# ArashMehraban/CeedPetscSolid

Hardware: AMD Instinct MI355X
Metric: MDoF/s for matrix-free Jacobian apply, p=4 hyperFS hex, 1/2/4/8 GPU (higher is better)
Workload: dtype f64; 1 GPU; config 4: hyperFS, hollow cylinder 10x110x90 = 99000 hex per GPU (stand-in for cylinder8_99Ke_4ss_us.exo), degree 4, Q=5, clamped ends, Jacobian apply y=J(u)x; global_dofs=19429080, elements_per_gpu=99000, ldofs_per_gpu=19537320, halo_dofs_rank0=0, assembly=pipelined: 2 segments on 2 streams, last segment 16384 elements, schedule=static, partition=single GPU

## Files before the change

ceedpetscsolid_amd/csrc/ceed_core.cpp:

```cpp
#include "ceed_impl.hpp"
#include "kernels_pointblock.hpp"

using namespace cps;

static int g_err_return = 0;
static thread_local char g_err_msg[1024] = "";

int ceed_error(const char *fmt, ...) {
  va_list ap;
  va_start(ap, fmt);
  vsnprintf(g_err_msg, sizeof g_err_msg, fmt, ap);
  va_end(ap);
  if (!g_err_return) {
    fprintf(stderr, "[ceed mi355x] error: %s\n", g_err_msg);
    abort();
  }
  return 1;
}
extern "C" int CeedXSetErrorReturn(int enable) { g_err_return = enable; return 0; }
extern "C" const char *CeedXLastError(void) { return g_err_msg; }

static CeedVector_private s_vec_active, s_vec_none;
static CeedElemRestriction_private s_rstr_none;
static CeedBasis_private s_basis_colloc;
static CeedQFunction_private s_qf_none;
static CeedRequest s_req_immediate, s_req_ordered;
extern "C" {
const CeedVector CEED_VECTOR_ACTIVE = &s_vec_active;
const CeedVector CEED_VECTOR_NONE = &s_vec_none;
const CeedElemRestriction CEED_ELEMRESTRICTION_NONE = &s_rstr_none;
const CeedBasis CEED_BASIS_COLLOCATED = &s_basis_colloc;
const CeedQFunction CEED_QFUNCTION_NONE = &s_qf_none;
CeedRequest *const CEED_REQUEST_IMMEDIATE = &s_req_immediate;
CeedRequest *const CEED_REQUEST_ORDERED = &s_req_ordered;
const CeedInt CEED_STRIDES_BACKEND[3] = {-1, -1, -1};
const char *const CeedMemTypes[] = {"host", "device"};
}

static int env_int(const char *name, int dflt) { const char *e = getenv(name); return e && *e ? atoi(e) : dflt; }
static bool env_is(const char *name, const char *val) { const char *e = getenv(name); return e && !strcmp(e, val); }

extern "C" int CeedInit(const char *resource, Ceed *ceed) {
  if (!resource || strncmp(resource, "/gpu/hip", 8))
    return ceed_error("this library serves /gpu/hip/mi355x only (got '%s'); there is no CPU path",
                      resource ? resource : "(null)");
  int ndev = 0;
  hipError_t e = hipGetDeviceCount(&ndev);
  if (e != hipSuccess || ndev < 1)
    return ceed_error("no HIP device visible (%s): the MI355X backend cannot run",
                      e != hipSuccess ? hipGetErrorString(e) : "device count 0");
  Ceed c = new Ceed_private;
  c->resource = "/gpu/hip/mi355x";
  HIPCHK(hipGetDevice(&c->device));
  CeedOptions &o = c->opt;
  o.recompute_geo = !env_is("CEED_MI355X_GEO", "0");
  o.direct_interior = !env_is("CEED_MI355X_DIRECT", "0");
  o.affine_geo = !env_is("CEED_MI355X_AFFINE", "0");
  o.swept_geo = !env_is("CEED_MI355X_SWEPT", "0");
  o.derived_state = !env_is("CEED_MI355X_DERIVED", "0");
  if (env_is("CEED_MI355X_ASSEMBLE", "serial")) o.pipe_segments = 0;
  else { const int ps = env_int("CEED_MI355X_PIPE_SEGMENTS", 0); o.pipe_segments = ps >= 2 ? std::min(ps, 16) : -1; }
  o.pipe_mb = std::max(0, env_int("CEED_MI355X_PIPE_MB", o.pipe_mb));
  o.pipe_min_total_rounds = std::max(0, env_int("CEED_MI355X_PIPE_MIN_TOTAL", o.pipe_min_total_rounds));
  o.pipe_min_rounds = std::max(0, env_int("CEED_MI355X_PIPE_MIN_ROUNDS", o.pipe_min_rounds));
  o.pencil_waves = std::max(0, env_int("CEED_MI355X_PENCIL_WAVES", 0));
  o.ovl_mode = env_int("CEED_MI355X_OVL_MODE", o.ovl_mode);
  o.ovl_groups0 = std::max(0, env_int("CEED_MI355X_OVL_G0", o.ovl_groups0));
  o.ovl_groups1 = std::max(0, env_int("CEED_MI355X_OVL_G1", o.ovl_groups1));
  o.comm_priority = env_int("CEED_MI355X_COMM_PRIO", o.comm_priority);
  o.comm_inline = env_int("CEED_MI355X_COMM_INLINE", o.comm_inline);
  o.fold_pack = env_int("CEED_MI355X_FOLD_PACK", o.fold_pack);
  *ceed = c;
  return 0;
}
void ceed_ref(Ceed c) { c->refcount++; }
int (*g_rccl_comm_destroy)(void *) = nullptr;
static void ceed_free_parked(Ceed c) {
  for (void *p : c->parked) (void)hipFree(p);
  c->parked.clear();
}
void ceed_retire(Ceed c, void *p) {
  if (!p) return;
  if (c->capturing || c->live_graphs > 0) c->parked.push_back(p);
  else { (void)hipStreamSynchronize(c->stream); (void)hipFree(p); }
}
void ceed_unref(Ceed c) {
  if (--c->refcount > 0) return;
  if (c->comm) {
    if (c->comm_stream) (void)hipStreamSynchronize(c->comm_stream);
    if (g_rccl_comm_destroy) g_rccl_comm_destroy(c->comm);
  }
  if (c->comm_stream) (void)hipStreamDestroy(c->comm_stream);
  if (c->capture_stream) (void)hipStreamDestroy(c->capture_stream);
  if (c->side_stream) (void)hipStreamDestroy(c->side_stream);
  c->evec.release();
  ceed_free_parked(c);
  if (c->ev_fork) (void)hipEventDestroy(c->ev_fork);
  if (c->ev_join) (void)hipEventDestroy(c->ev_join);
  for (hipEvent_t ev : c->ev_seg) if (ev) (void)hipEventDestroy(ev);
  if (c->h_scalar) (void)hipHostFree(c->h_scalar);
  delete c;
}
int ceed_need_side_stream(Ceed c) {
  if (c->side_stream) return 0;
  HIPCHK(hipStreamCreateWithFlags(&c->side_stream, hipStreamNonBlocking));
  HIPCHK(hipEventCreateWithFlags(&c->ev_fork, hipEventDisableTiming));
  HIPCHK(hipEventCreateWithFlags(&c->ev_join, hipEventDisableTiming));
  return 0;
}
extern "C" int CeedDestroy(Ceed *ceed) {
  if (!ceed || !*ceed) return 0;
  ceed_unref(*ceed);
  *ceed = nullptr;
  return 0;
}
extern "C" int CeedGetResource(Ceed ceed, const char **resource) { *resource = ceed->resource.c_str(); return 0; }
extern "C" int CeedGetPreferredMemType(Ceed, CeedMemType *type) { *type = CEED_MEM_DEVICE; return 0; }
extern "C" int CeedXSetStream(Ceed ceed, void *s) { ceed->stream = (hipStream_t)s; return 0; }
extern "C" int CeedXSynchronize(Ceed ceed) {
  if (ceed->capturing) return ceed_error("CeedXSynchronize during graph capture");
  HIPCHK(hipStreamSynchronize(ceed->stream));
  return 0;
}
extern "C" int CeedXClockProbe(Ceed ceed, int spin_us, double *ghz) {
  if (ceed->capturing) return ceed_error("CeedXClockProbe during graph capture");
  if (spin_us < 1 || spin_us > 1000000) return ceed_error("CeedXClockProbe: 1 us ... 1 s");
  struct Stream { hipStream_t s = nullptr; ~Stream() { if (s) (void)hipStreamDestroy(s); } } ps;
  DevArray<long long> d;
  long long h[2] = {0, 0};
  HIPCHK(hipStreamCreateWithFlags(&ps.s, hipStreamNonBlocking));
  CHK(d.alloc(nullptr, 2));
  HIPCHK(launch_clock_probe(d.get(), spin_us, ps.s));
  HIPCHK(hipMemcpyAsync(h, d.get(), sizeof h, hipMemcpyDeviceToHost, ps.s));
  HIPCHK(hipStreamSynchronize(ps.s));
  *ghz = h[1] > 0 ? (double)h[0] / ((double)h[1] * 10.0) : 0.;
  return 0;
}
static void release_capture_deps(Ceed ceed) {
  std::vector<GraphDep> deps;
  deps.swap(ceed->capture_deps);
  for (GraphDep &d : deps) { CeedVector v = d.v; (void)CeedVectorDestroy(&v); }
}
extern "C" int CeedXGraphBeginCapture(Ceed ceed) {
  if (ceed->capturing) return ceed_error("graph capture already in progress");
  HIPCHK(hipStreamSynchronize(ceed->stream));
  if (!ceed->capture_stream) HIPCHK(hipStreamCreateWithFlags(&ceed->capture_stream, hipStreamNonBlocking));
  ceed->saved_stream = ceed->stream;
  ceed->stream = ceed->capture_stream;
  HIPCHK(hipStreamBeginCapture(ceed->stream, hipStreamCaptureModeRelaxed));
  ceed->capturing = true;
  release_capture_deps(ceed);
  return 0;
}
extern "C" int CeedXGraphEndCapture(Ceed ceed, CeedXGraph *graph) {
// ... 363 lines not shown
```

ceedpetscsolid_amd/csrc/ceed_impl.hpp:

```cpp
#pragma once
#include <ceed.h>
#include <hip/hip_runtime_api.h>

#include <algorithm>
#include <cmath>
#include <cstdarg>
#include <cstdio>
#include <cstdlib>
#include <cstring>
#include <memory>
#include <string>
#include <vector>

#include "dev_array.hpp"
#include "kernels.hpp"

int ceed_error(const char *fmt, ...);
#define CHK(x) do { int ierr_ = (x); if (ierr_) return ierr_; } while (0)
#define HIPCHK(x) do { hipError_t e_ = (x); if (e_ != hipSuccess) \
  return ceed_error("%s failed: %s (%s:%d)", #x, hipGetErrorString(e_), __FILE__, __LINE__); } while (0)

struct CeedOptions {
  bool recompute_geo = true;
  bool direct_interior = true;
  bool derived_state = true;
  bool affine_geo = true;
  bool swept_geo = true;
  int pipe_segments = -1;
  int pipe_mb = 0;
  int pipe_min_total_rounds = 20;
  int pipe_min_rounds = 4;
  int pencil_waves = 0;
  int ovl_mode = 0;
  int ovl_groups0 = 1, ovl_groups1 = 0;
  int fold_pack = 1;
  int comm_inline = 1;
  int comm_priority = 0;
};

struct GraphDep { CeedVector v; const double *geo; const double *derived; };
struct Ceed_private {
  int refcount = 1;
  std::string resource;
  hipStream_t stream = nullptr;
  int device = 0;
  CeedOptions opt;
  DevArray<double> evec;
  std::vector<void *> parked;
  int live_graphs = 0;
  hipStream_t side_stream = nullptr;
  hipEvent_t ev_fork = nullptr, ev_join = nullptr;
  hipEvent_t ev_seg[16] = {nullptr};
  void *comm = nullptr;
  int comm_rank = 0, comm_size = 1;
  hipStream_t comm_stream = nullptr;
  DevArray<double> d_scalar;
  double *h_scalar = nullptr;
  DevArray<int> d_pb_bad;
  hipStream_t capture_stream = nullptr, saved_stream = nullptr;
  bool capturing = false;
  std::vector<GraphDep> capture_deps;
};
struct CeedXGraph_private {
  std::vector<GraphDep> deps;
  Ceed ceed = nullptr;
  hipGraph_t graph = nullptr;
  hipGraphExec_t exec = nullptr;
  size_t nodes = 0;
};

struct CeedVector_private {
  Ceed ceed = nullptr;
  int refcount = 1;
  CeedInt length = 0;
  double *h = nullptr, *d = nullptr;
  uint64_t version = 0;
  bool h_owned = false, d_owned = false;
  bool h_valid = false, d_valid = false;
  DevArray<double> geo;
  DevArray<double> geo_aff;
  DevArray<double> geo_swept;
  int geo_axis = 0;
  int geo_nelem = 0, geo_Q = 0;
  double geo_qref[cps::MAXN1D] = {0}, geo_qwt[cps::MAXN1D] = {0};
  DevArray<double> derived;
  bool derived_valid = false;
  int derived_nelem = 0, derived_Q3 = 0;
  double derived_nu = 0., derived_E = 0.;
};

struct RowMap {
  std::vector<uint32_t> h_node_off;
  DevArray<uint32_t> d_rowptr, d_cols, d_node_off;
  int nrows = 0;
  cps::NodeMap view() const { return cps::NodeMap{d_rowptr.get(), d_cols.get(), d_node_off.get(), nrows, 0}; }
};
struct CsrMap : RowMap {
  bool built = false, full_cover = false;
  int nprio = 0, nskipped = 0;
  std::vector<uint32_t> h_rowptr, h_cols;
};
struct PipeMap : RowMap {
  int E = 0, req_seg = 0, waves = 0, mb = 0;
  const CsrMap *base = nullptr;
  int nseg = 0;
  std::vector<int> elem_bound, row_bound;
};

struct CeedElemRestriction_private {
  Ceed ceed = nullptr;
  int refcount = 1;
  CeedInt nelem = 0, elemsize = 0, ncomp = 0, compstride = 0, lsize = 0;
  bool strided = false, backend_strides = true;
  CeedInt strides[3] = {0, 0, 0};
  std::vector<CeedInt> h_offsets;
  DevArray<uint32_t> d_offsets;
  CsrMap csr;
  CsrMap csr_shell;
  std::vector<std::unique_ptr<PipeMap>> pipes;
  int interior_private = 0;
  DevArray<uint32_t> d_int_off;
  int int_per_elem = 0;
};

struct CeedBasis_private {
  Ceed ceed = nullptr;
  int refcount = 1;
  CeedInt dim = 3, ncomp = 0, P1d = 0, Q1d = 0;
  CeedQuadMode qmode = CEED_GAUSS;
  std::vector<double> interp1d, grad1d, qref1d, qweight1d, colo1d;
};

struct QFField { std::string name; CeedInt size; CeedEvalMode emode; };

struct CeedQFunction_private {
  Ceed ceed = nullptr;
  int refcount = 1;
  CeedQFunctionUser f = nullptr;
  std::string source, name;
  int kind = cps::QF_NONE;
  void *ctx = nullptr;
  size_t ctxsize = 0;
  CeedInt identity_size = 0;
  std::vector<QFField> in, out;
};

struct OpField { bool set = false; CeedElemRestriction rstr = nullptr; CeedBasis basis = nullptr; CeedVector vec = nullptr; };

enum PlanKind { PLAN_NONE = 0, PLAN_FUSED_GRAD, PLAN_SETUP_GEO, PLAN_PROLONG, PLAN_RESTRICT, PLAN_COORD, PLAN_ENERGY };

struct CeedXHalo_private;

struct CeedOperator_private {
  Ceed ceed = nullptr;
  int refcount = 1;
  CeedQFunction qf = nullptr;
  std::vector<OpField> in, out;
  bool composite = false;
  std::vector<CeedOperator> sub;
  int plan = PLAN_NONE;
  int i_active = -1, i_qdata = -1, i_state = -1, i_weight = -1, o_active = -1, o_state = -1, o_qdata = -1;
  cps::BasisTables tables;
  double eo[6][cps::EO_TAB];
  std::string kernel_name;
  bool kernel_fused = false;
  std::string kernel_name_full;
  int geo_mode = 0;
  DevArray<uint32_t> d_off_flagged;
  std::vector<std::pair<const RowMap *, DevArray<unsigned char>>> row_flags;
  struct PackFold { const RowMap *M; CeedXHalo H; long serial; DevArray<uint32_t> d_ptr, d_slot; bool ok; };
  std::vector<PackFold> pack_folds;
  std::vector<unsigned char> h_mask;
  int mask_mode = 0;
  CeedVector scale = nullptr;
  std::vector<unsigned char> h_mask_fine;
  DevArray<uint32_t> d_own_f;
  bool own_full_cover = false;
  DevArray<double> d_w;
  bool w_ready = false, w_unit = false;
  CeedVector w_scale = nullptr;
  uint64_t w_version = 0;
  int ovl_lead = 0;
  CsrMap ovl_csr;
  long ovl_halo_checked = 0;
  bool timing = false;
  std::vector<std::pair<hipEvent_t, hipEvent_t>> events;
  double ms_accum = 0.;
  int64_t launches = 0;
  int launch_info[4] = {0, 0, 0, 0};
};

void ceed_ref(Ceed c);
void ceed_unref(Ceed c);
int ceed_need_evec(Ceed c, size_t len);
int ceed_need_side_stream(Ceed c);
int dev_zero(Ceed c, double *p, size_t n);
int vec_dev(CeedVector v, bool write, double **p);
void vec_drop_geo(CeedVector v);

int build_csr(CeedElemRestriction r, CsrMap &M, const unsigned char *prio, int skipP = 0);
bool rstr_interior_private(CeedElemRestriction r, int P);
int build_interior_list(CeedElemRestriction r, int P);
int get_pipe(CeedElemRestriction r, const CsrMap &M, int E, int per_elem, int req_seg, int waves, int mb_per_segment, PipeMap **out);

struct HaloNeighbour { int rank = 0, n = 0, offset = 0; };
struct CeedXHalo_private {
  Ceed ceed = nullptr;
  long serial = 0;
  std::vector<HaloNeighbour> nb;
  int total = 0;
  DevArray<uint32_t> d_idx;
  std::vector<uint32_t> h_idx;
  DevArray<double> send, recv;
  int ndst = 0;
  DevArray<uint32_t> d_dst, d_uptr, d_uslot;
  hipEvent_t packed = nullptr, arrived = nullptr;
  hipStream_t arrived_on = nullptr;
  bool in_flight = false;
  CeedInt lsize_min = 0;
};
int halo_pack_and_send(CeedXHalo H, const double *py, hipStream_t pack_stream);
int halo_send(CeedXHalo H, hipStream_t pack_stream);
int halo_wait_arrivals(CeedXHalo H, hipStream_t s);
cps::HaloUnpackArgs halo_unpack_args(CeedXHalo H);

static inline bool is_offsets(CeedElemRestriction r) { return r && r != CEED_ELEMRESTRICTION_NONE && !r->strided; }
static inline bool is_strided(CeedElemRestriction r) { return r && r != CEED_ELEMRESTRICTION_NONE && r->strided; }
```

ceedpetscsolid_amd/csrc/ceed_restriction.cpp:

```cpp
#include "ceed_impl.hpp"

using namespace cps;

extern "C" int CeedElemRestrictionCreate(Ceed ceed, CeedInt nelem, CeedInt elemsize, CeedInt ncomp,
                                         CeedInt compstride, CeedInt lsize, CeedMemType mtype,
                                         CeedCopyMode, const CeedInt *offsets, CeedElemRestriction *rstr) {
  if (mtype != CEED_MEM_HOST) return ceed_error("restriction offsets are expected in host memory (setuplibceed.c:235)");
  if ((uint32_t)lsize > OFF_MASK) return ceed_error("L-vector of %d entries exceeds the 2^29 offset range of this backend", lsize);
  const size_t n = (size_t)nelem * elemsize;
  for (size_t i = 0; i < n; i++) {
    const long last = (long)offsets[i] + (long)(ncomp - 1) * compstride;
    if (offsets[i] < 0 || last >= lsize)
      return ceed_error("restriction offset %zu = %d out of range [0,%d)", i, offsets[i], lsize);
  }
  CeedElemRestriction r = new CeedElemRestriction_private;
  r->ceed = ceed; ceed_ref(ceed);
  r->nelem = nelem; r->elemsize = elemsize; r->ncomp = ncomp; r->compstride = compstride; r->lsize = lsize;
  r->h_offsets.assign(offsets, offsets + n);
  static_assert(sizeof(CeedInt) == sizeof(uint32_t), "the offsets are uploaded as they are (checked non-negative above)");
  const int ierr = r->d_offsets.upload(ceed, (const uint32_t *)offsets, n);
  if (ierr) { (void)CeedElemRestrictionDestroy(&r); return ierr; }
  *rstr = r;
  return 0;
}
extern "C" int CeedElemRestrictionCreateStrided(Ceed ceed, CeedInt nelem, CeedInt elemsize, CeedInt ncomp,
                                                CeedInt lsize, const CeedInt strides[3], CeedElemRestriction *rstr) {
  if ((long)nelem * elemsize * ncomp > lsize) return ceed_error("strided restriction larger than its L-vector");
  CeedElemRestriction r = new CeedElemRestriction_private;
  r->ceed = ceed; ceed_ref(ceed);
  r->nelem = nelem; r->elemsize = elemsize; r->ncomp = ncomp; r->lsize = lsize;
  r->strided = true;
  r->backend_strides = strides[0] < 0;
  if (r->backend_strides) { r->strides[0] = 1; r->strides[1] = elemsize; r->strides[2] = elemsize * ncomp; }
  else {
    memcpy(r->strides, strides, sizeof r->strides);
    if (!(strides[0] == 1 && strides[1] == elemsize && strides[2] == elemsize * ncomp)) {
      (void)CeedElemRestrictionDestroy(&r);
      return ceed_error("only the [elem][comp][node] strided layout is supported on /gpu/hip/mi355x");
    }
  }
  *rstr = r;
  return 0;
}
extern "C" int CeedElemRestrictionCreateVector(CeedElemRestriction r, CeedVector *lvec, CeedVector *evec) {
  if (lvec) CHK(CeedVectorCreate(r->ceed, r->lsize, lvec));
  if (evec) CHK(CeedVectorCreate(r->ceed, r->nelem * r->elemsize * r->ncomp, evec));
  return 0;
}
extern "C" int CeedElemRestrictionApply(CeedElemRestriction r, CeedTransposeMode tmode, CeedVector u,
                                        CeedVector ru, CeedRequest *) {
  hipStream_t s = r->ceed->stream;
  double *pu, *pv;
  CHK(vec_dev(u, false, &pu));
  CHK(vec_dev(ru, true, &pv));
  if (r->strided) {
    const size_t n = (size_t)r->nelem * r->elemsize * r->ncomp;
    if (tmode == CEED_NOTRANSPOSE) HIPCHK(hipMemcpyAsync(pv, pu, n * sizeof(double), hipMemcpyDeviceToDevice, s));
    else HIPCHK(launch_axpby(pv, 1., pu, 1., n, s));
    return 0;
  }
  if (tmode == CEED_NOTRANSPOSE) HIPCHK(launch_rstr_gather(r->d_offsets.get(), r->nelem, r->elemsize, r->ncomp, r->compstride, pu, pv, s));
  else HIPCHK(launch_rstr_scatter_add(r->d_offsets.get(), r->nelem, r->elemsize, r->ncomp, r->compstride, pu, pv, s));
  return 0;
}
extern "C" int CeedElemRestrictionGetMultiplicity(CeedElemRestriction r, CeedVector mult) {
  if (r->strided) return CeedVectorSetValue(mult, 1.);
  CHK(CeedVectorSetValue(mult, 0.));
  HIPCHK(launch_multiplicity(r->d_offsets.get(), r->nelem, r->elemsize, r->ncomp, r->compstride, mult->d, r->ceed->stream));
  return 0;
}
extern "C" int CeedElemRestrictionDestroy(CeedElemRestriction *rstr) {
  if (!rstr || !*rstr) return 0;
  CeedElemRestriction r = *rstr;
  *rstr = nullptr;
  if (r == CEED_ELEMRESTRICTION_NONE) return 0;
  if (--r->refcount > 0) return 0;
  Ceed c = r->ceed;
  delete r;
  ceed_unref(c);
  return 0;
}

int build_csr(CeedElemRestriction r, CsrMap &M, const unsigned char *prio, int skipP) {
  if (M.built) return 0;
  if (r->ceed->capturing)
    return ceed_error("first apply of an operator during graph capture: its restriction's transpose map is built on the host; "
                      "apply the operator once before recording");
  const size_t n = r->h_offsets.size();
  std::vector<uint32_t> cnt((size_t)r->lsize + 1, 0u);
  for (size_t i = 0; i < n; i++) cnt[(size_t)r->h_offsets[i]]++;
  M.nskipped = 0;
  if (skipP > 0)
    for (size_t i = 0; i < n; i++)
      if (node_is_element_interior((int)(i % (size_t)r->elemsize), skipP)) { cnt[(size_t)r->h_offsets[i]] = 0; M.nskipped++; }
  std::vector<uint32_t> slot((size_t)r->lsize, 0xFFFFFFFFu);
  std::vector<uint32_t> &rowptr = M.h_rowptr, &cols = M.h_cols;
  M.h_node_off.clear(); rowptr.clear();
  rowptr.push_back(0u);
  M.nprio = 0;
  for (int pass = prio ? 0 : 1; pass < 2; pass++)
    for (CeedInt o = 0; o < r->lsize; o++) {
      if (!cnt[o]) continue;
      if (prio && ((prio[o] != 0) != (pass == 0))) continue;
      slot[o] = (uint32_t)M.h_node_off.size();
      M.h_node_off.push_back((uint32_t)o);
      rowptr.push_back(rowptr.back() + cnt[o]);
      if (prio && pass == 0) M.nprio++;
    }
  const int nn = (int)M.h_node_off.size();
  std::vector<uint32_t> cursor(rowptr.begin(), rowptr.end() - 1);
  cols.assign(rowptr.back() ? rowptr.back() : 1, 0u);
  for (size_t i = 0; i < n; i++) {
    const uint32_t sl = slot[(size_t)r->h_offsets[i]];
    if (sl == 0xFFFFFFFFu) continue;
    const size_t e = i / (size_t)r->elemsize; const int ln = (int)(i % (size_t)r->elemsize);
    cols[cursor[sl]++] = skipP > 0 ? (uint32_t)(e * (size_t)element_shell_size(skipP) + (size_t)node_shell_rank(ln, skipP)) : (uint32_t)i;
  }
  M.nrows = nn;
  M.full_cover = ((size_t)nn + (size_t)M.nskipped) * (size_t)r->ncomp == (size_t)r->lsize;
  CHK(M.d_rowptr.upload(r->ceed, rowptr)); CHK(M.d_cols.upload(r->ceed, cols)); CHK(M.d_node_off.upload(r->ceed, M.h_node_off));
  M.built = true;
  return 0;
}
bool rstr_interior_private(CeedElemRestriction r, int P) {
  if (r->interior_private) return r->interior_private > 0;
  r->interior_private = -1;
  if (P < 3 || (size_t)P * P * P != (size_t)r->elemsize || r->ncomp != 3 || r->compstride != 1) return false;
  std::vector<unsigned char> cnt((size_t)r->lsize, 0);
  for (size_t i = 0; i < r->h_offsets.size(); i++) {
    unsigned char &c = cnt[(size_t)r->h_offsets[i]];
    if (c < 2) c++;
  }
  for (size_t i = 0; i < r->h_offsets.size(); i++)
    if (node_is_element_interior((int)(i % (size_t)r->elemsize), P) && cnt[(size_t)r->h_offsets[i]] != 1) return false;
  r->interior_private = 1;
  return true;
}

int build_interior_list(CeedElemRestriction r, int P) {
  if (r->d_int_off || P < 3) return 0;
  if (r->ceed->capturing) return ceed_error("first apply of an operator during graph capture: apply it once before recording");
  const int m = (P - 2) * (P - 2) * (P - 2);
  std::vector<uint32_t> lst((size_t)r->nelem * m);
  size_t k = 0;
  for (CeedInt e = 0; e < r->nelem; e++)
    for (int n = 0; n < r->elemsize; n++)
      if (node_is_element_interior(n, P)) lst[k++] = (uint32_t)r->h_offsets[(size_t)e * r->elemsize + n];
  CHK(r->d_int_off.upload(r->ceed, lst));
  r->int_per_elem = m;
  return 0;
}

int get_pipe(CeedElemRestriction r, const CsrMap &M, int E, int per_elem, int req_seg_in, int waves, int mb, PipeMap **out) {
  for (auto &p : r->pipes)
    if (p->E == E && p->req_seg == req_seg_in && p->waves == waves && p->mb == mb && p->base == &M) { *out = p.get(); return 0; }
  const CeedOptions &opt = r->ceed->opt;
  int req_seg = req_seg_in;
  const int ngroups = (r->nelem + E - 1) / E;
  const int min_rounds = opt.pipe_min_rounds;
  if (min_rounds > 0 && ngroups < opt.pipe_min_total_rounds * std::max(waves, 1)) req_seg = 1;
  else if (req_seg == 0) req_seg = std::max(2, std::min(16, (int)((double)r->nelem * per_elem * 24. / (1e6 * std::max(mb, 1)) + 0.5)));
  int nseg = min_rounds > 0 ? std::max(1, std::min(req_seg, ngroups / (min_rounds * std::max(waves, 1)))) : std::min(req_seg, std::max(1, ngroups));
  if (nseg >= 2 && r->ceed->capturing) { *out = nullptr; return 0; }
  std::unique_ptr<PipeMap> Gp(new PipeMap);
  PipeMap &G = *Gp;
  G.E = E; G.req_seg = req_seg_in; G.waves = waves; G.mb = mb; G.base = &M;
  if (nseg < 2) { G.nseg = 1; *out = Gp.get(); r->pipes.push_back(std::move(Gp)); return 0; }
  G.elem_bound.assign(1, 0);
  constexpr int last_rounds = 4;
  const long total_rounds = ngroups / std::max(waves, 1);
  std::vector<long> gb;
  if (min_rounds > 0 && total_rounds >= last_rounds + (long)(nseg - 1) * min_rounds) {
    long g = (long)ngroups - (long)last_rounds * waves;
    gb.push_back(g);
    const long per = (total_rounds - last_rounds) / (nseg - 1);
    for (int k = nseg - 2; k >= 1; k--) { g -= per * waves; gb.push_back(g); }
  } else {
    for (int k = nseg - 1; k >= 1; k--) {
      long g = (long)ngroups * k / nseg;
      const long up = (long)ngroups - (((long)ngroups - g) / waves) * waves;
      gb.push_back(min_rounds > 0 && up > 0 && up < ngroups ? up : g);
    }
  }
  for (auto it = gb.rbegin(); it != gb.rend(); ++it) {
    const int e = (int)std::min<long>((long)r->nelem, *it * E);
    if (e > G.elem_bound.back() && e < r->nelem) G.elem_bound.push_back(e);
  }
  G.elem_bound.push_back(r->nelem);
  nseg = (int)G.elem_bound.size() - 1;
  G.nseg = nseg;
  const int nn = M.nrows;
  const std::vector<uint32_t> &rowptr = M.h_rowptr, &cols = M.h_cols;
  std::vector<int> seg((size_t)nn);
  std::vector<uint32_t> cnt((size_t)nseg + 1, 0u);
  for (int i = 0; i < nn; i++) {
    const int elast = (int)(cols[rowptr[i + 1] - 1] / (uint32_t)per_elem);
    const int k = (int)(std::upper_bound(G.elem_bound.begin(), G.elem_bound.end(), elast) - G.elem_bound.begin()) - 1;
    seg[i] = k; cnt[(size_t)k + 1]++;
  }
  for (int k = 0; k < nseg; k++) cnt[k + 1] += cnt[k];
  G.row_bound.assign(cnt.begin(), cnt.end());
  std::vector<uint32_t> cursor(cnt.begin(), cnt.end() - 1), order((size_t)nn);
  for (int i = 0; i < nn; i++) order[cursor[seg[i]]++] = (uint32_t)i;
  std::vector<uint32_t> rp2((size_t)nn + 1, 0u), cols2(cols.size()), no2((size_t)(nn ? nn : 1));
  G.h_node_off.resize((size_t)nn);
  for (int j = 0; j < nn; j++) {
    const uint32_t i = order[j], len = rowptr[i + 1] - rowptr[i];
    for (uint32_t k = 0; k < len; k++) cols2[rp2[j] + k] = cols[rowptr[i] + k];
    rp2[j + 1] = rp2[j] + len;
    no2[j] = G.h_node_off[j] = M.h_node_off[i];
  }
  G.nrows = nn;
  CHK(G.d_rowptr.upload(r->ceed, rp2)); CHK(G.d_cols.upload(r->ceed, cols2)); CHK(G.d_node_off.upload(r->ceed, no2));
  *out = Gp.get();
  r->pipes.push_back(std::move(Gp));
  return 0;
}
```

ceedpetscsolid_amd/csrc/kernel_node_sum.hpp:

```cpp
#pragma once
#include "kernels_common.hpp"

namespace cps {

CPS_DEV void node_sum3(const uint32_t *rowptr, const uint32_t *cols, const double *evec, int r, double &a0, double &a1, double &a2) {
  const uint32_t k0 = rowptr[r], k1 = rowptr[r + 1];
  for (uint32_t k = k0; k < k1; k += 4) {
    uint32_t c[4];
#pragma unroll
    for (int j = 0; j < 4; j++) c[j] = cols[k + j < k1 ? k + j : k1 - 1];
    double v[4][3];
#pragma unroll
    for (int j = 0; j < 4; j++) {
      const double *p = evec + (size_t)c[j] * 3;
      v[j][0] = p[0]; v[j][1] = p[1]; v[j][2] = p[2];
    }
#pragma unroll
    for (int j = 0; j < 4; j++)
      if (k + j < k1) { a0 += v[j][0]; a1 += v[j][1]; a2 += v[j][2]; }
  }
}

CPS_DEV void halo_unpack_add(const HaloUnpackArgs &un, double *y, int first, int stride) {
  for (int u = first; u < un.n; u += stride) {
    double v = y[un.dst[u]];
    for (uint32_t k = un.ptr[u]; k < un.ptr[u + 1]; k++) v += un.recv[un.slot[k]];
    y[un.dst[u]] = v;
  }
}

CPS_DEV void cheb_dof_regs(double rbase, bool has_t, double ti, bool store_r, size_t i, double dinv_i, double d_i, double x_i, double *x, double *d,
                           double *r, double c1, double c2, int assign_x) {
#pragma clang fp contract(off)
  const double ri = has_t ? rbase - ti : rbase;
  if (store_r) r[i] = ri;
  double di = (c1 * dinv_i) * ri;
  if (c2 != 0.) di = __builtin_fma(c2, d_i, di);
  d[i] = di;
  x[i] = assign_x ? di : x_i + di;
}
CPS_DEV void cheb_dof(double rbase, bool has_t, double ti, bool store_r, size_t i, double *x, double *d, double *r, const double *dinv,
                      double c1, double c2, int assign_x) {
  cheb_dof_regs(rbase, has_t, ti, store_r, i, dinv[i], c2 != 0. ? d[i] : 0., assign_x ? 0. : x[i], x, d, r, c1, c2, assign_x);
}

}
```

ceedpetscsolid_amd/csrc/kernels.hpp:

```cpp
#pragma once
#include <hip/hip_runtime_api.h>
#include <stdint.h>

namespace cps {

enum QFKind : int {
  QF_NONE = 0,
  QF_SETUP_GEO,
  QF_LINELAS,
  QF_HYPERSS_F,
  QF_HYPERSS_DF,
  QF_HYPERFS_F,
  QF_HYPERFS_DF,
  QF_IDENTITY,
  QF_CONST_FORCE,
  QF_MMS_FORCE,
  QF_MMS_TRUE,
  QF_ENERGY_LINELAS,
  QF_ENERGY_HYPERSS,
  QF_ENERGY_HYPERFS,
  QF_DIAG_LINELAS,
  QF_DIAG_HYPERSS,
  QF_DIAG_HYPERFS,
  QF_HYPERFS_DF_DS,
// ... 57 lines not shown
#ifdef __HIPCC__
__host__ __device__
#endif
static inline int node_shell_rank(int n, int P) {
  const int m = P - 2, i = n % P, j = (n / P) % P, k = n / (P * P);
  if (k == 0) return j * P + i;
  if (k == P - 1) return P * P + j * P + i;
  if (j == 0) return 2 * P * P + (k - 1) * P + i;
  if (j == P - 1) return 2 * P * P + P * m + (k - 1) * P + i;
  if (i == 0) return 2 * P * P + 2 * P * m + (k - 1) * m + (j - 1);
  return 2 * P * P + 2 * P * m + m * m + (k - 1) * m + (j - 1);
}
#ifdef __HIPCC__
__host__ __device__
#endif
static inline int element_shell_size(int P) { return P * P * P - (P > 2 ? (P - 2) * (P - 2) * (P - 2) : 0); }

struct TransferArgs {
  const uint32_t *off_c;
  const uint32_t *own_f;
  const double *x;
  double *y;
  const double *w_f;
  int nelem;
  int mask_c, mask_f;
  int add;
  double *evec;
};
hipError_t launch_transfer_weights(double *w, const double *scale, size_t n, int *n_not_unit, hipStream_t s);

constexpr int GEO_NCOEF = 21;
hipError_t launch_geo_coeffs(const uint32_t *off_x, const double *xcoord, double *geo, int nelem, hipStream_t s);
constexpr int GEO_NAFF = 10;
hipError_t launch_geo_affine(const double *geo, double *aff, int nelem, int *n_not_affine, hipStream_t s);
constexpr int GEO_NSWEPT = 8;
hipError_t launch_geo_swept(const double *geo, double *sw, int nelem, int *count, int axis, hipStream_t s);

struct SetupGeoArgs {
  const uint32_t *off_x;
  const double *xcoord;
  double *qdata;
  int nelem;
};

struct DiagArgs {
  const uint32_t *offsets;
  const double *qdata, *state_in;
  int nelem;
  int mask_in, mask_out;
  double nu, E, lambda, TwoMu;
  double *evec;
};

struct StateArgs {
  const uint32_t *offsets;
  const double *x;
  const double *qdata;
  double *state_out;
  int nelem;
  int mask_in;
};

hipError_t launch_fused_grad(int P, int Q, int qf, const BasisTables &t, const FusedGradArgs &a, FusedLaunch l, hipStream_t s, const char **name);
hipError_t launch_transfer(int Pc, int Pf, bool prolong, const BasisTables &t, const TransferArgs &a,
                           hipStream_t s, const char **name);
hipError_t launch_setup_geo(int Q, const BasisTables &t, const SetupGeoArgs &a, hipStream_t s,
                            const char **name);
hipError_t launch_diag(int P, int Q, int qf, const BasisTables &t, const DiagArgs &a, hipStream_t s,
                       const char **name);
hipError_t launch_state_at_points(int Pf, int Qc, const BasisTables &t, const StateArgs &a, hipStream_t s,
                                  const char **name);

constexpr int pencil_inst_parts(int Q) { return Q == 8 ? 4 : (Q == 7 ? 2 : 1); }
constexpr int pencil_group_elems(int Q) { return Q <= 2 ? 8 : (Q <= 4 ? 4 : (Q == 5 ? 2 : 1)); }
constexpr int PENCIL_MINW = 2;
constexpr int pencil_lds_bytes(int Q) { return (pencil_group_elems(Q) * (9 * Q * Q * Q + (Q == 5 ? 5 : 1) + GEO_NCOEF) + 2 * Q) * 8; }
constexpr int pencil_waves_per_cu(int Q) {
  const int by_lds = (160 * 1024) / pencil_lds_bytes(Q); return by_lds < 1 ? 1 : (by_lds > 4 * PENCIL_MINW ? 4 * PENCIL_MINW : by_lds);
}

struct NodeMap {
  const uint32_t *rowptr, *cols, *node_off;
  int nnodes, row0;
  NodeMap rows(int first, int n) const { return NodeMap{rowptr, cols, node_off, n, first}; }
};
struct HaloUnpackArgs { const uint32_t *dst, *ptr, *slot; const double *recv; int n; };
struct HaloPackFold { const uint32_t *ptr, *slot; double *send; };
hipError_t launch_assemble(const NodeMap &m, const unsigned char *flags, const double *evec, double *y, int add, hipStream_t s,
                           const HaloUnpackArgs *unpack = nullptr, const HaloPackFold *pack = nullptr);

enum EpilogueKind : int { EPI_NONE = 0, EPI_CHEB = 1, EPI_RESID = 2 };
struct EpilogueArgs {
  int kind;
  const double *t;
  const uint32_t *int_off;
  int n_int;
  double *x, *d, *r;
  const double *r0, *dinv;
  double c1, c2;
  int assign_x;
  double *w;
  const double *b;
};
hipError_t launch_assemble_epi(const NodeMap &m, const unsigned char *flags, const double *evec, const EpilogueArgs &ep, hipStream_t s);

struct CoordOpArgs {
  const uint32_t *off_x;
  const double *xcoord;
  const uint32_t *off_u;
  double *y;
  const double *qdata;
  int nelem, Q, Pout, mode;
  double ctx[3];
  double bx[MAXN1D * 2];
  double bu[MAXN1D * MAXN1D];
};
hipError_t launch_coord_op(const CoordOpArgs &a, hipStream_t s);
struct EnergyOpArgs {
  const uint32_t *off_u;
  const double *u;
  const uint32_t *off_e;
  double *y;
  const double *qdata;
  int nelem, Q, P, model;
  int diag;
  double nu, E;
  double interp[MAXN1D * MAXN1D], grad[MAXN1D * MAXN1D];
  double interp_e[MAXN1D * MAXN1D];
};
hipError_t launch_energy_op(const EnergyOpArgs &a, hipStream_t s);

hipError_t launch_halo_pack(const uint32_t *idx, int n, const double *y, double *buf, hipStream_t s);
hipError_t launch_halo_unpack_add(const HaloUnpackArgs &u, double *y, hipStream_t s);

hipError_t launch_csr_sum(const uint32_t *slotptr, const uint32_t *perm, const double *coo, double *vals, int nnz,
                          const uint32_t *unit_diag_slot, int n_unit, hipStream_t s);
hipError_t launch_csr_spmv_stream(const uint32_t *row_block, int nblocks, const uint32_t *rowptr, const uint32_t *cols, const double *vals,
                                  const double *x, double *y, hipStream_t s);
hipError_t launch_csr_diag(const uint32_t *diag_slot_of_row, const double *vals, double *d, int nrows, hipStream_t s);
hipError_t launch_csr_spgemm(const uint32_t *l_rowptr, const uint32_t *l_cols, const double *l_vals, const uint32_t *r_rowptr,
                             const uint32_t *r_cols, const double *r_vals, const uint32_t *c_rowptr, const uint32_t *c_cols, double *c_vals,
                             int nrows, hipStream_t s, int dense_ncols = 0, int max_row_c = 0);
hipError_t launch_dense_spd_inverse(double *A, int n, double *scratch , int *info, hipStream_t s);

hipError_t launch_set_value(double *v, size_t n, double val, hipStream_t s);
hipError_t launch_waxpby(double *w, double a, const double *x, double b, const double *y, size_t n, hipStream_t s);
hipError_t launch_cheb_update(double *x, double *d, double *r, const double *r0, const double *t, const double *dinv, double c1, double c2,
                              int assign_x, size_t n, hipStream_t s);
hipError_t launch_reciprocal(double *v, size_t n, hipStream_t s);
hipError_t launch_pointwise_mult(double *w, const double *x, const double *y, size_t n, hipStream_t s);
hipError_t launch_axpby(double *y, double a, const double *x, double b, size_t n, hipStream_t s);
hipError_t launch_masked_copy(double *dst, const double *src, const unsigned char *mask, size_t n,
                              hipStream_t s);
hipError_t launch_rstr_gather(const uint32_t *off, int nelem, int elemsize, int ncomp, int compstride,
                              const double *l, double *e, hipStream_t s);
hipError_t launch_rstr_scatter_add(const uint32_t *off, int nelem, int elemsize, int ncomp,
                                   int compstride, const double *e, double *l, hipStream_t s);
hipError_t launch_multiplicity(const uint32_t *off, int nelem, int elemsize, int ncomp, int compstride,
                               double *l, hipStream_t s);
hipError_t launch_dot(const double *x, const double *y, const double *w, size_t n, double *result_dev,
                      hipStream_t s, double *out = nullptr);
hipError_t launch_scalar_div(double *sc, int dst, int num, int den, double scale, hipStream_t s);
hipError_t launch_axpby_dev(double *y, const double *sc, int ia, double sa, const double *x, int ib, double sb, size_t n, hipStream_t s);

}
```

ceedpetscsolid_amd/csrc/kernels_assemble.hip:

```cpp
#include <algorithm>
#include "kernel_node_sum.hpp"

namespace cps {

__global__ void k_rstr(const uint32_t *off, size_t total, int elemsize, int ncomp, int compstride,
                       const double *src, double *dst, int mode) {
  for (size_t i = blockIdx.x * (size_t)blockDim.x + threadIdx.x; i < total; i += (size_t)gridDim.x * blockDim.x) {
    const size_t n = i % elemsize, ec = i / elemsize, c = ec % ncomp, e = ec / ncomp;
    const size_t li = (size_t)(off[e * elemsize + n] & OFF_MASK) + c * (size_t)compstride;
    if (mode == 0) dst[i] = src[li];
    else if (mode == 1) atomic_add_f64(dst + li, src[i]);
    else atomic_add_f64(dst + li, 1.0);
  }
}
__global__ void k_assemble(const uint32_t *rowptr, const uint32_t *cols, const uint32_t *node_off,
                           const unsigned char *flags, const double *evec, double *y, int nnodes, int add, int nb_rows,
                           const HaloUnpackArgs un, const HaloPackFold pk) {
  if ((int)blockIdx.x >= nb_rows) {
    halo_unpack_add(un, y, ((int)blockIdx.x - nb_rows) * blockDim.x + threadIdx.x, ((int)gridDim.x - nb_rows) * blockDim.x);
    return;
  }
  for (int r = blockIdx.x * blockDim.x + threadIdx.x; r < nnodes; r += nb_rows * blockDim.x) {
    double a0 = 0., a1 = 0., a2 = 0.;
    node_sum3(rowptr, cols, evec, r, a0, a1, a2);
    const unsigned fl = flags ? flags[r] : 0u;
    double *dst = y + (node_off[r] & OFF_MASK);
    if (fl & 1u) a0 = 0.;
    if (fl & 2u) a1 = 0.;
    if (fl & 4u) a2 = 0.;
    if (add) { a0 += dst[0]; a1 += dst[1]; a2 += dst[2]; }
    dst[0] = a0; dst[1] = a1; dst[2] = a2;
    if (pk.ptr)
      for (uint32_t k = pk.ptr[r]; k < pk.ptr[r + 1]; k++) {
        const uint32_t e = pk.slot[k], cmp = e >> 30;
        pk.send[e & 0x3FFFFFFFu] = cmp == 0 ? a0 : (cmp == 1 ? a1 : a2);
      }
  }
}

__global__ void k_assemble_epi(const uint32_t *rowptr, const uint32_t *cols, const uint32_t *node_off, const unsigned char *flags,
                               const double *evec, int nnodes, int nb_rows, const EpilogueArgs ep) {
  if ((int)blockIdx.x >= nb_rows) {
    const size_t n = (size_t)ep.n_int * 3;
    for (size_t u = ((size_t)blockIdx.x - nb_rows) * blockDim.x + threadIdx.x; u < n; u += ((size_t)gridDim.x - nb_rows) * blockDim.x) {
      const size_t i = (size_t)(ep.int_off[u / 3] & OFF_MASK) + u % 3;
      const double ti = ep.t[i];
      if (ep.kind == EPI_CHEB) cheb_dof(ep.r0 ? ep.r0[i] : ep.r[i], true, ti, ep.r != nullptr, i, ep.x, ep.d, ep.r, ep.dinv, ep.c1, ep.c2, ep.assign_x);
      else ep.w[i] = ep.b[i] - ti;
    }
    return;
  }
  const int lane = threadIdx.x & 63;
  const int wave = (int)((blockIdx.x * blockDim.x + threadIdx.x) >> 6), nwaves = (int)((nb_rows * blockDim.x) >> 6);
  for (int row0 = wave * 64; row0 < nnodes; row0 += nwaves * 64) {
    const int r = row0 + lane;
    const bool live = r < nnodes;
    const uint32_t off = live ? (node_off[r] & OFF_MASK) : 0u;
    size_t idx[3];
    bool ok[3];
    double s0[3], s1[3], s2[3], s3[3];
#pragma unroll
    for (int q = 0; q < 3; q++) {
      const int j = 64 * q + lane, src = j / 3, c = j % 3;
      idx[q] = (size_t)__shfl(off, src, 64) + c;
      ok[q] = row0 + src < nnodes;
      s0[q] = s1[q] = s2[q] = s3[q] = 0.;
      if (ok[q]) {
        if (ep.kind == EPI_CHEB) {
          s0[q] = ep.r0 ? ep.r0[idx[q]] : ep.r[idx[q]]; s1[q] = ep.dinv[idx[q]];
          s2[q] = ep.c2 != 0. ? ep.d[idx[q]] : 0.; s3[q] = ep.assign_x ? 0. : ep.x[idx[q]];
        } else s0[q] = ep.b[idx[q]];
      }
    }
    double a0 = 0., a1 = 0., a2 = 0.;
    if (live) {
      node_sum3(rowptr, cols, evec, r, a0, a1, a2);
      const unsigned fl = flags ? flags[r] : 0u;
      if (fl & 1u) a0 = 0.;
      if (fl & 2u) a1 = 0.;
      if (fl & 4u) a2 = 0.;
    }
#pragma unroll
    for (int q = 0; q < 3; q++) {
      const int j = 64 * q + lane, src = j / 3, c = j % 3;
      const double t0 = __shfl(a0, src, 64), t1 = __shfl(a1, src, 64), t2 = __shfl(a2, src, 64);
      const double ti = c == 0 ? t0 : (c == 1 ? t1 : t2);
      if (!ok[q]) continue;
      if (ep.kind == EPI_CHEB) cheb_dof_regs(s0[q], true, ti, ep.r != nullptr, idx[q], s1[q], s2[q], s3[q], ep.x, ep.d, ep.r, ep.c1, ep.c2, ep.assign_x);
      else ep.w[idx[q]] = s0[q] - ti;
    }
  }
}
hipError_t launch_assemble_epi(const NodeMap &m, const unsigned char *flags, const double *evec, const EpilogueArgs &ep, hipStream_t s) {
  if (m.nnodes <= 0 && ep.n_int <= 0) return hipSuccess;
  constexpr int AB = 256;
  const unsigned nb_rows = (unsigned)((std::max(m.nnodes, 0) + AB - 1) / AB);
  const unsigned nb_int = (unsigned)std::min<size_t>(((size_t)std::max(ep.n_int, 0) * 3 + AB - 1) / AB, 4096);
  hipLaunchKernelGGL(k_assemble_epi, dim3(nb_rows + nb_int), dim3(AB), 0, s, m.rowptr + m.row0, m.cols, m.node_off + m.row0,
                     flags ? flags + m.row0 : nullptr, evec, m.nnodes, (int)nb_rows, ep);
  return hipGetLastError();
}
hipError_t launch_assemble(const NodeMap &m, const unsigned char *flags, const double *evec, double *y, int add, hipStream_t s,
                           const HaloUnpackArgs *unpack, const HaloPackFold *pack) {
  const int nun = unpack ? unpack->n : 0;
  if (m.nnodes <= 0 && nun <= 0) return hipSuccess;
  constexpr int AB = 256;
  const unsigned nb_rows = (unsigned)((std::max(m.nnodes, 0) + AB - 1) / AB);
  const unsigned nb_un = (unsigned)std::min((nun + AB - 1) / AB, 1024);
  hipLaunchKernelGGL(k_assemble, dim3(nb_rows + nb_un), dim3(AB), 0, s, m.rowptr + m.row0, m.cols, m.node_off + m.row0,
                     flags ? flags + m.row0 : nullptr, evec, y, m.nnodes, add, (int)nb_rows,
                     unpack ? *unpack : HaloUnpackArgs{nullptr, nullptr, nullptr, nullptr, 0},
                     pack ? HaloPackFold{pack->ptr + m.row0, pack->slot, pack->send} : HaloPackFold{nullptr, nullptr, nullptr});
  return hipGetLastError();
}

__global__ void k_halo_pack(const uint32_t *idx, int n, const double *y, double *buf) {
  for (int i = blockIdx.x * blockDim.x + threadIdx.x; i < n; i += gridDim.x * blockDim.x) buf[i] = y[idx[i]];
}
__global__ void k_halo_unpack_add(const HaloUnpackArgs un, double *y) {
  halo_unpack_add(un, y, blockIdx.x * blockDim.x + threadIdx.x, gridDim.x * blockDim.x);
}
hipError_t launch_halo_pack(const uint32_t *idx, int n, const double *y, double *buf, hipStream_t s) {
  return launch_stream(k_halo_pack, (size_t)std::max(n, 0), s, idx, n, y, buf);
}
hipError_t launch_halo_unpack_add(const HaloUnpackArgs &u, double *y, hipStream_t s) {
  return launch_stream(k_halo_unpack_add, (size_t)std::max(u.n, 0), s, u, y);
}

static hipError_t rstr(const uint32_t *off, int nelem, int elemsize, int ncomp, int compstride,
                       const double *src, double *dst, int mode, hipStream_t s) {
  const size_t total = (size_t)nelem * elemsize * ncomp;
  return launch_stream(k_rstr, total, s, off, total, elemsize, ncomp, compstride, src, dst, mode);
}
hipError_t launch_rstr_gather(const uint32_t *off, int nelem, int elemsize, int ncomp, int compstride,
                              const double *l, double *e, hipStream_t s) {
  return rstr(off, nelem, elemsize, ncomp, compstride, l, e, 0, s);
}
hipError_t launch_rstr_scatter_add(const uint32_t *off, int nelem, int elemsize, int ncomp, int compstride,
                                   const double *e, double *l, hipStream_t s) {
  return rstr(off, nelem, elemsize, ncomp, compstride, e, l, 1, s);
}
hipError_t launch_multiplicity(const uint32_t *off, int nelem, int elemsize, int ncomp, int compstride,
                               double *l, hipStream_t s) {
  return rstr(off, nelem, elemsize, ncomp, compstride, nullptr, l, 2, s);
}

}
```

Measured before the change: 48140 MDoF/s.

## Encode CSR node-sum rows as shared stencil patterns with base position

Result: faster. 48960 MDoF/s, median of 6 (+1.7%).

```diff
diff --git a/ceedpetscsolid_amd/csrc/ceed_core.cpp b/ceedpetscsolid_amd/csrc/ceed_core.cpp
--- a/ceedpetscsolid_amd/csrc/ceed_core.cpp
+++ b/ceedpetscsolid_amd/csrc/ceed_core.cpp
@@ -70,6 +70,8 @@
   o.comm_priority = env_int("CEED_MI355X_COMM_PRIO", o.comm_priority);
   o.comm_inline = env_int("CEED_MI355X_COMM_INLINE", o.comm_inline);
   o.fold_pack = env_int("CEED_MI355X_FOLD_PACK", o.fold_pack);
+  o.row_code = !env_is("CEED_MI355X_ROWMAP", "plain");
+  o.row_code_max = std::max(0, env_int("CEED_MI355X_ROWCODE_MAX", o.row_code_max));
   *ceed = c;
   return 0;
 }
diff --git a/ceedpetscsolid_amd/csrc/ceed_impl.hpp b/ceedpetscsolid_amd/csrc/ceed_impl.hpp
--- a/ceedpetscsolid_amd/csrc/ceed_impl.hpp
+++ b/ceedpetscsolid_amd/csrc/ceed_impl.hpp
@@ -36,6 +36,8 @@
   int fold_pack = 1;
   int comm_inline = 1;
   int comm_priority = 0;
+  bool row_code = true;
+  int row_code_max = 4096;
 };
 
 struct GraphDep { CeedVector v; const double *geo; const double *derived; };
@@ -93,7 +95,14 @@
   std::vector<uint32_t> h_node_off;
   DevArray<uint32_t> d_rowptr, d_cols, d_node_off;
   int nrows = 0;
-  cps::NodeMap view() const { return cps::NodeMap{d_rowptr.get(), d_cols.get(), d_node_off.get(), nrows, 0}; }
+  DevArray<uint32_t> d_pos0, d_stencil;
+  DevArray<uint16_t> d_sid;
+  int nstencils = 0, nescape = 0;
+  cps::NodeMap view() const {
+    cps::NodeMap m{d_rowptr.get(), d_cols.get(), d_node_off.get(), nrows, 0};
+    m.pos0 = d_pos0.get(); m.sid = d_sid.get(); m.stencil = d_stencil.get();
+    return m;
+  }
 };
 struct CsrMap : RowMap {
   bool built = false, full_cover = false;
@@ -199,6 +208,7 @@
 void vec_drop_geo(CeedVector v);
 
 int build_csr(CeedElemRestriction r, CsrMap &M, const unsigned char *prio, int skipP = 0);
+int upload_row_code(Ceed c, RowMap &M, const std::vector<uint32_t> &rowptr, const std::vector<uint32_t> &cols);
 bool rstr_interior_private(CeedElemRestriction r, int P);
 int build_interior_list(CeedElemRestriction r, int P);
 int get_pipe(CeedElemRestriction r, const CsrMap &M, int E, int per_elem, int req_seg, int waves, int mb_per_segment, PipeMap **out);
diff --git a/ceedpetscsolid_amd/csrc/ceed_restriction.cpp b/ceedpetscsolid_amd/csrc/ceed_restriction.cpp
--- a/ceedpetscsolid_amd/csrc/ceed_restriction.cpp
+++ b/ceedpetscsolid_amd/csrc/ceed_restriction.cpp
@@ -1,4 +1,5 @@
 #include "ceed_impl.hpp"
+#include "row_code.hpp"
 
 using namespace cps;
 
@@ -78,6 +79,16 @@
   Ceed c = r->ceed;
   delete r;
   ceed_unref(c);
+  return 0;
+}
+
+int upload_row_code(Ceed c, RowMap &M, const std::vector<uint32_t> &rowptr, const std::vector<uint32_t> &cols) {
+  if (!c->opt.row_code) return 0;
+  const RowCode code = row_code_encode(rowptr, cols, c->opt.row_code_max);
+  static_assert(sizeof(RowStencil) == 8 * sizeof(uint32_t), "a stencil is uploaded as eight words");
+  CHK(M.d_pos0.upload(c, code.pos0)); CHK(M.d_sid.upload(c, code.sid));
+  CHK(M.d_stencil.upload(c, (const uint32_t *)code.table.data(), code.table.size() * 8));
+  M.nstencils = (int)code.table.size(); M.nescape = (int)code.nescape;
   return 0;
 }
 
@@ -119,6 +130,7 @@
   M.nrows = nn;
   M.full_cover = ((size_t)nn + (size_t)M.nskipped) * (size_t)r->ncomp == (size_t)r->lsize;
   CHK(M.d_rowptr.upload(r->ceed, rowptr)); CHK(M.d_cols.upload(r->ceed, cols)); CHK(M.d_node_off.upload(r->ceed, M.h_node_off));
+  CHK(upload_row_code(r->ceed, M, rowptr, cols));
   M.built = true;
   return 0;
 }
@@ -212,6 +224,7 @@
   }
   G.nrows = nn;
   CHK(G.d_rowptr.upload(r->ceed, rp2)); CHK(G.d_cols.upload(r->ceed, cols2)); CHK(G.d_node_off.upload(r->ceed, no2));
+  CHK(upload_row_code(r->ceed, G, rp2, cols2));
   *out = Gp.get();
   r->pipes.push_back(std::move(Gp));
   return 0;
diff --git a/ceedpetscsolid_amd/csrc/kernel_node_sum.hpp b/ceedpetscsolid_amd/csrc/kernel_node_sum.hpp
--- a/ceedpetscsolid_amd/csrc/kernel_node_sum.hpp
+++ b/ceedpetscsolid_amd/csrc/kernel_node_sum.hpp
@@ -18,6 +18,40 @@
 #pragma unroll
     for (int j = 0; j < 4; j++)
       if (k + j < k1) { a0 += v[j][0]; a1 += v[j][1]; a2 += v[j][2]; }
+  }
+}
+
+constexpr int ROWCODE_LANE_MAXC = 8;
+struct RowCodeView { const uint32_t *pos0; const uint16_t *sid; const uint32_t *stencil; };
+CPS_DEV void node_sum3_coded(const RowCodeView &rc, const uint32_t *rowptr, const uint32_t *cols, const double *evec, int r, double &a0, double &a1, double &a2) {
+  const uint32_t s = rc.sid[r];
+  uint32_t p0 = rc.pos0[r];
+  asm volatile("" : "+v"(p0));
+  if (s == 0xFFFFu) { node_sum3(rowptr, cols, evec, r, a0, a1, a2); return; }
+  const uint4 *st = reinterpret_cast<const uint4 *>(rc.stencil) + 2 * (size_t)s;
+  uint4 lo = st[0], hi = st[1];
+  asm volatile("" : "+v"(lo.x), "+v"(lo.y), "+v"(lo.z), "+v"(lo.w), "+v"(hi.x), "+v"(hi.y), "+v"(hi.z), "+v"(hi.w));
+  const uint32_t n = lo.x;
+  const uint32_t d[ROWCODE_LANE_MAXC] = {0u, lo.y, lo.z, lo.w, hi.x, hi.y, hi.z, hi.w};
+  const bool more = n > 4u;
+  double v[ROWCODE_LANE_MAXC][3] = {};
+#pragma unroll
+  for (int j = 0; j < 4; j++) {
+    const double *p = evec + (size_t)(p0 + d[j]) * 3;
+    v[j][0] = p[0]; v[j][1] = p[1]; v[j][2] = p[2];
+  }
+  if (more) {
+#pragma unroll
+    for (int j = 4; j < 8; j++) {
+      const double *p = evec + (size_t)(p0 + d[j]) * 3;
+      v[j][0] = p[0]; v[j][1] = p[1]; v[j][2] = p[2];
+    }
+  }
+#pragma unroll
+  for (int j = 0; j < 8; j++) {
+    const bool take = (uint32_t)j < n;
+    const double t0 = a0 + v[j][0], t1 = a1 + v[j][1], t2 = a2 + v[j][2];
+    a0 = take ? t0 : a0; a1 = take ? t1 : a1; a2 = take ? t2 : a2;
   }
 }
 
diff --git a/ceedpetscsolid_amd/csrc/kernels.hpp b/ceedpetscsolid_amd/csrc/kernels.hpp
--- a/ceedpetscsolid_amd/csrc/kernels.hpp
+++ b/ceedpetscsolid_amd/csrc/kernels.hpp
@@ -163,7 +163,10 @@
 struct NodeMap {
   const uint32_t *rowptr, *cols, *node_off;
   int nnodes, row0;
-  NodeMap rows(int first, int n) const { return NodeMap{rowptr, cols, node_off, n, first}; }
+  const uint32_t *pos0 = nullptr;
+  const uint16_t *sid = nullptr;
+  const uint32_t *stencil = nullptr;
+  NodeMap rows(int first, int n) const { NodeMap m = *this; m.row0 = first; m.nnodes = n; return m; }
 };
 struct HaloUnpackArgs { const uint32_t *dst, *ptr, *slot; const double *recv; int n; };
 struct HaloPackFold { const uint32_t *ptr, *slot; double *send; };
diff --git a/ceedpetscsolid_amd/csrc/kernels_assemble.hip b/ceedpetscsolid_amd/csrc/kernels_assemble.hip
--- a/ceedpetscsolid_amd/csrc/kernels_assemble.hip
+++ b/ceedpetscsolid_amd/csrc/kernels_assemble.hip
@@ -15,14 +15,15 @@
 }
 __global__ void k_assemble(const uint32_t *rowptr, const uint32_t *cols, const uint32_t *node_off,
                            const unsigned char *flags, const double *evec, double *y, int nnodes, int add, int nb_rows,
-                           const HaloUnpackArgs un, const HaloPackFold pk) {
+                           const HaloUnpackArgs un, const HaloPackFold pk, const RowCodeView rc) {
   if ((int)blockIdx.x >= nb_rows) {
     halo_unpack_add(un, y, ((int)blockIdx.x - nb_rows) * blockDim.x + threadIdx.x, ((int)gridDim.x - nb_rows) * blockDim.x);
     return;
   }
   for (int r = blockIdx.x * blockDim.x + threadIdx.x; r < nnodes; r += nb_rows * blockDim.x) {
     double a0 = 0., a1 = 0., a2 = 0.;
-    node_sum3(rowptr, cols, evec, r, a0, a1, a2);
+    if (rc.sid) node_sum3_coded(rc, rowptr, cols, evec, r, a0, a1, a2);
+    else node_sum3(rowptr, cols, evec, r, a0, a1, a2);
     const unsigned fl = flags ? flags[r] : 0u;
     double *dst = y + (node_off[r] & OFF_MASK);
     if (fl & 1u) a0 = 0.;
@@ -39,7 +40,7 @@
 }
 
 __global__ void k_assemble_epi(const uint32_t *rowptr, const uint32_t *cols, const uint32_t *node_off, const unsigned char *flags,
-                               const double *evec, int nnodes, int nb_rows, const EpilogueArgs ep) {
+                               const double *evec, int nnodes, int nb_rows, const EpilogueArgs ep, const RowCodeView rc) {
   if ((int)blockIdx.x >= nb_rows) {
     const size_t n = (size_t)ep.n_int * 3;
     for (size_t u = ((size_t)blockIdx.x - nb_rows) * blockDim.x + threadIdx.x; u < n; u += ((size_t)gridDim.x - nb_rows) * blockDim.x) {
@@ -74,7 +75,8 @@
     }
     double a0 = 0., a1 = 0., a2 = 0.;
     if (live) {
-      node_sum3(rowptr, cols, evec, r, a0, a1, a2);
+      if (rc.sid) node_sum3_coded(rc, rowptr, cols, evec, r, a0, a1, a2);
+      else node_sum3(rowptr, cols, evec, r, a0, a1, a2);
       const unsigned fl = flags ? flags[r] : 0u;
       if (fl & 1u) a0 = 0.;
       if (fl & 2u) a1 = 0.;
@@ -91,13 +93,16 @@
     }
   }
 }
+static RowCodeView row_code_view(const NodeMap &m) {
+  return m.sid ? RowCodeView{m.pos0 + m.row0, m.sid + m.row0, m.stencil} : RowCodeView{nullptr, nullptr, nullptr};
+}
 hipError_t launch_assemble_epi(const NodeMap &m, const unsigned char *flags, const double *evec, const EpilogueArgs &ep, hipStream_t s) {
   if (m.nnodes <= 0 && ep.n_int <= 0) return hipSuccess;
   constexpr int AB = 256;
   const unsigned nb_rows = (unsigned)((std::max(m.nnodes, 0) + AB - 1) / AB);
   const unsigned nb_int = (unsigned)std::min<size_t>(((size_t)std::max(ep.n_int, 0) * 3 + AB - 1) / AB, 4096);
   hipLaunchKernelGGL(k_assemble_epi, dim3(nb_rows + nb_int), dim3(AB), 0, s, m.rowptr + m.row0, m.cols, m.node_off + m.row0,
-                     flags ? flags + m.row0 : nullptr, evec, m.nnodes, (int)nb_rows, ep);
+                     flags ? flags + m.row0 : nullptr, evec, m.nnodes, (int)nb_rows, ep, row_code_view(m));
   return hipGetLastError();
 }
 hipError_t launch_assemble(const NodeMap &m, const unsigned char *flags, const double *evec, double *y, int add, hipStream_t s,
@@ -110,7 +115,8 @@
   hipLaunchKernelGGL(k_assemble, dim3(nb_rows + nb_un), dim3(AB), 0, s, m.rowptr + m.row0, m.cols, m.node_off + m.row0,
                      flags ? flags + m.row0 : nullptr, evec, y, m.nnodes, add, (int)nb_rows,
                      unpack ? *unpack : HaloUnpackArgs{nullptr, nullptr, nullptr, nullptr, 0},
-                     pack ? HaloPackFold{pack->ptr + m.row0, pack->slot, pack->send} : HaloPackFold{nullptr, nullptr, nullptr});
+                     pack ? HaloPackFold{pack->ptr + m.row0, pack->slot, pack->send} : HaloPackFold{nullptr, nullptr, nullptr},
+                     row_code_view(m));
   return hipGetLastError();
 }
 
diff --git a/ceedpetscsolid_amd/csrc/row_code.hpp b/ceedpetscsolid_amd/csrc/row_code.hpp
--- /dev/null
+++ b/ceedpetscsolid_amd/csrc/row_code.hpp
@@ -0,0 +1,83 @@
+#pragma once
+#include <stdint.h>
+
+#include <cstddef>
+#include <map>
+#include <vector>
+
+namespace cps {
+
+constexpr int ROWCODE_MAXC = 8;
+constexpr uint16_t ROWCODE_ESCAPE = 0xFFFFu;
+constexpr int ROWCODE_MAX_DEFAULT = 4096;
+
+struct RowStencil {
+  uint32_t count;
+  uint32_t dist[ROWCODE_MAXC - 1];
+};
+static_assert(sizeof(RowStencil) == 32, "the kernels read a stencil as two 16-byte halves");
+
+struct RowCode {
+  std::vector<uint32_t> pos0;
+  std::vector<uint16_t> sid;
+  std::vector<RowStencil> table;
+  size_t nescape = 0;
+};
+
+inline RowCode row_code_encode(const std::vector<uint32_t> &rowptr, const std::vector<uint32_t> &cols, int max_stencils = ROWCODE_MAX_DEFAULT) {
+  RowCode c;
+  const size_t nrows = rowptr.empty() ? 0 : rowptr.size() - 1;
+  const size_t limit = (size_t)(max_stencils < 0 ? 0 : (max_stencils > (int)ROWCODE_ESCAPE ? (int)ROWCODE_ESCAPE : max_stencils));
+  c.pos0.assign(nrows, 0u);
+  c.sid.assign(nrows, ROWCODE_ESCAPE);
+  std::map<std::vector<uint32_t>, uint16_t> ids;
+  std::vector<uint32_t> key;
+  for (size_t r = 0; r < nrows; r++) {
+    const uint32_t k0 = rowptr[r], k1 = rowptr[r + 1];
+    bool ok = k1 >= k0 && k1 - k0 <= (uint32_t)ROWCODE_MAXC;
+    key.assign(1, ok ? k1 - k0 : 0u);
+    for (uint32_t k = k0 + 1; ok && k < k1; k++) {
+      if (cols[k] < cols[k0]) ok = false;
+      else key.push_back(cols[k] - cols[k0]);
+    }
+    if (ok) {
+      auto it = ids.find(key);
+      if (it == ids.end()) {
+        if (c.table.size() >= limit) ok = false;
+        else {
+          RowStencil s{};
+          s.count = key[0];
+          for (int j = 0; j < ROWCODE_MAXC - 1; j++)
+            s.dist[j] = (size_t)j + 1 < key.size() ? key[(size_t)j + 1] : (key.size() > 1 ? key.back() : 0u);
+          it = ids.emplace(key, (uint16_t)c.table.size()).first;
+          c.table.push_back(s);
+        }
+      }
+      if (ok) { c.sid[r] = it->second; c.pos0[r] = k1 > k0 ? cols[k0] : 0u; }
+    }
+    if (!ok) c.nescape++;
+  }
+  return c;
+}
+
+inline bool row_code_decode(const RowCode &c, const std::vector<uint32_t> &rowptr, const std::vector<uint32_t> &cols,
+                            std::vector<uint32_t> &rowptr_out, std::vector<uint32_t> &cols_out) {
+  const size_t nrows = rowptr.empty() ? 0 : rowptr.size() - 1;
+  rowptr_out.assign(1, 0u);
+  cols_out.clear();
+  if (c.pos0.size() != nrows || c.sid.size() != nrows) return false;
+  for (size_t r = 0; r < nrows; r++) {
+    if (c.sid[r] == ROWCODE_ESCAPE) {
+      for (uint32_t k = rowptr[r]; k < rowptr[r + 1]; k++) cols_out.push_back(cols[k]);
+    } else {
+      if ((size_t)c.sid[r] >= c.table.size()) return false;
+      const RowStencil &s = c.table[c.sid[r]];
+      if (s.count > (uint32_t)ROWCODE_MAXC) return false;
+      for (uint32_t j = 0; j < s.count; j++) cols_out.push_back(c.pos0[r] + (j ? s.dist[j - 1] : 0u));
+    }
+    rowptr_out.push_back((uint32_t)cols_out.size());
+  }
+  return true;
+}
+
+}
```
